# leopard-ai/betty

Hardware: AMD Instinct MI355X
Metric: hypergradient-steps/sec (CG K=20, 10M inner params) (higher is better)
Workload: dtype f32

## Files before the change

betty_amd/_native.py:

```python
from __future__ import annotations

import ctypes
import os
from ctypes import POINTER, c_char_p, c_double, c_float, c_int, c_int32, c_int64, c_size_t, c_void_p

_HERE = os.path.dirname(os.path.abspath(__file__))
LIB_PATH = os.environ.get("BHG_LIB") or os.path.join(_HERE, "csrc", "libbhg.so")
AB_LIB_PATH = os.environ.get("BHG_AB_LIB") or os.path.join(_HERE, "csrc", "libbhg_ab.so")

BHG_CHUNK_ELEMS = 4096
BHG_FLAT_ALIGN = 64
BHG_CG_AUTO, BHG_CG_STREAM, BHG_CG_RESIDENT = 0, 1, 2
BHG_CG_GLOBAL_CHAIN, BHG_CG_GLOBAL_UPDATE, BHG_CG_GLOBAL_DOTS = 0, 1, 2
BHG_CG_FX_BEGIN, BHG_CG_FX_CHAIN, BHG_CG_FX_GRAM, BHG_CG_FX_END = 0, 1, 2, 3


class NativeLibraryError(RuntimeError):
    """libbhg.so is missing or a call into it failed."""


class Chunk(ctypes.Structure):

    _fields_ = [
        ("flat_off", c_int64),
# ... 98 lines not shown
        c_int,
        [c_void_p, c_void_p, c_void_p, c_void_p, c_void_p, c_void_p, c_void_p, c_int, c_int, c_int, c_float, c_float, c_int, c_int, c_void_p],
    ),
    "bhg_logreg_neumann_solve": (
        c_int,
        [c_void_p, c_void_p, c_void_p, c_void_p, c_void_p, c_void_p, c_void_p, c_int, c_int, c_int, c_float, c_float, c_int, c_int, c_void_p],
    ),
    "bhg_mlp_partial_floats": (c_size_t, [POINTER(Mlp)]),
    "bhg_mlp_hvp": (c_int, [POINTER(Mlp), _PP, _PP, c_void_p]),
    "bhg_mlp_hvp_mode": (c_int, [POINTER(Mlp), _PP, _PP, c_int, c_void_p]),
    "bhg_mlp_supports_native_prepare": (c_int, [POINTER(Mlp)]),
    "bhg_mlp_forward": (c_int, [POINTER(Mlp), _PP, c_void_p, c_void_p, c_void_p]),
    "bhg_mlp_backward": (c_int, [POINTER(Mlp), c_void_p, c_void_p]),
    "bhg_mlp_mixed_coeff": (c_int, [POINTER(Mlp), _PP, c_void_p, c_void_p, c_void_p]),
    "bhg_mlp_supports_fused_solve": (c_int, [POINTER(Mlp)]),
    "bhg_mlp_fused_ws_bytes": (c_size_t, [POINTER(Mlp)]),
    "bhg_mlp_cg_solve": (
        c_int,
        [POINTER(Mlp), c_void_p, c_void_p, c_void_p, POINTER(c_int64), _CH, c_int, c_int, c_float, c_float, c_void_p,
         c_void_p, c_size_t, c_void_p],
    ),
    "bhg_mlp_cg_state_mask": (ctypes.c_uint64, [POINTER(Mlp), c_int]),
    "bhg_mlp_cg_solve_rhs": (
        c_int,
        [POINTER(Mlp), c_void_p, c_void_p, c_void_p, POINTER(c_int64), _CH, c_int, c_int, c_float, c_float, c_void_p,
         c_void_p, c_size_t, _PP, c_void_p],
    ),
    "bhg_mlp_cg_global_phase": (
        c_int,
        [POINTER(Mlp), c_void_p, c_void_p, c_void_p, POINTER(c_int64), _CH, c_int, c_int, c_int, c_int, c_int, c_void_p, c_float,
         c_float, c_void_p, c_void_p, c_size_t, c_void_p],
    ),
    "bhg_mlp_fx_supported": (c_int, [POINTER(Mlp), c_int]),
    "bhg_mlp_fx_ws_bytes": (c_size_t, [POINTER(Mlp), c_int]),
    "bhg_mlp_fx_const_floats": (c_size_t, [POINTER(Mlp)]),
    "bhg_mlp_fx_slab_floats": (c_size_t, [POINTER(Mlp)]),
    "bhg_mlp_fx_scal_doubles": (c_size_t, [POINTER(Mlp)]),
    "bhg_mlp_cg_fx_phase": (
        c_int,
        [POINTER(Mlp), _PP, c_int, c_int, c_int, c_int, c_int, c_void_p, c_void_p, c_void_p, c_float, c_float, c_void_p, c_size_t,
         c_void_p, c_size_t, c_void_p],
    ),
    "bhg_mlp_neumann_fx_phase": (
        c_int,
        [POINTER(Mlp), _PP, c_int, c_int, c_int, c_int, c_int, c_void_p, c_void_p, c_void_p, c_float, c_float, c_void_p, c_size_t,
         c_void_p, c_size_t, c_void_p],
    ),
    "bhg_mlp_cg_mixed_coeff": (c_int, [POINTER(Mlp), c_void_p, c_void_p, c_float, c_void_p, c_size_t, c_void_p]),
    "bhg_mlp_timeout_flag_dev": (c_void_p, [POINTER(Mlp), c_void_p]),
    "bhg_mlp_stage_batch": (c_int, [POINTER(Mlp), c_void_p, c_void_p, c_void_p, c_void_p]),
    "bhg_mlp_supports_packed_prepare": (c_int, [POINTER(Mlp)]),
    "bhg_mlp_forward_packed": (c_int, [POINTER(Mlp), _PP, c_void_p, c_void_p, c_void_p, c_size_t, c_void_p]),
    "bhg_mlp_backward_packed": (c_int, [POINTER(Mlp), c_void_p, c_void_p, c_size_t, c_void_p]),
    "bhg_mwn_max_hidden": (c_int, []),
    "bhg_mlp_fd_ws_bytes": (c_size_t, [POINTER(c_int), c_int, c_int]),
    "bhg_mlp_fd_forward": (
        c_int,
        [c_void_p, c_void_p, c_int, POINTER(c_int), c_int, _PP, _PP, c_void_p, c_int, c_void_p, c_void_p, c_void_p, c_size_t, c_void_p],
    ),
    "bhg_mwn_fd_vjp": (
        c_int,
        [c_void_p, c_void_p, c_int, c_void_p, c_void_p, c_void_p, c_void_p, c_int, c_void_p, c_int, c_void_p, c_void_p, c_void_p, c_void_p,
         c_void_p],
    ),
    "bhg_quad_fd": (c_int, [_PP, _PP, _PP, c_int, _CH, c_int, c_void_p, c_float, c_int, c_int, c_int, c_void_p]),
    "bhg_mwn_forward": (c_int, [c_void_p, c_int, c_void_p, c_void_p, c_void_p, c_void_p, c_int, c_void_p, c_void_p, c_void_p]),
    "bhg_mwn_backward": (
        c_int,
        [c_void_p, c_void_p, c_int, c_void_p, c_void_p, c_void_p, c_void_p, c_int, c_float, c_void_p, c_void_p, c_void_p, c_void_p, c_void_p],
    ),
    "bhg_mlp_neumann_solve": (
        c_int,
        [POINTER(Mlp), c_void_p, c_void_p, c_void_p, POINTER(c_int64), c_int, c_float, c_float, c_void_p, c_size_t, POINTER(c_int), c_void_p],
    ),
    "bhg_mlp_wsk_launches": (c_int64, []),
    "bhg_mlp_hoist_launches": (c_int64, []),
    "bhg_mlp_proj_iterations": (c_int64, []),
    "bhg_mlp_lin_launches": (c_int64, []),
    "bhg_mlp_neumann_mixed_coeff": (c_int, [POINTER(Mlp), _PP, c_void_p, c_void_p, c_float, c_int, c_int, c_void_p, c_size_t, c_void_p]),
    "bhg_mlp_plan_describe": (c_int, [POINTER(Mlp), c_int, c_int, ctypes.c_char_p, c_size_t]),
    "bhg_copy2d": (c_int, [c_void_p, c_int64, c_void_p, c_int64, c_int64, c_int64, c_void_p]),
    "bhg_bn_ws_bytes": (c_size_t, [c_int]),
    "bhg_bn_backward_vjp": (
        c_int,
        [c_void_p, c_void_p, c_void_p, c_void_p, c_void_p, c_void_p, c_void_p, c_void_p, c_int, c_int, c_int, c_void_p, c_void_p, c_void_p,
         c_void_p, c_size_t, c_void_p],
    ),
}

_libs = {}
_current = [None]


_PY_ENV = {"BHG_LIB", "BHG_AB_LIB", "BHG_HVP_GRAPH", "BHG_ALL_RANKS_ON_GPU0"}
_warned_env = [False]


def _warn_legacy_env() -> None:
    if _warned_env[0]:
        return
    _warned_env[0] = True
    stale = sorted(k for k in os.environ if k.startswith("BHG_") and k not in _PY_ENV)
    if stale:
        import warnings

        warnings.warn("betty_amd: environment variable(s) " + ", ".join(stale) + " are IGNORED — libbhg reads no environment variable. "
# ... 101 lines not shown
```

betty_amd/csrc/bhg_common.hpp:

```cpp
#pragma once
#include <hip/hip_runtime.h>
#include <stdint.h>
#include <stddef.h>
#include <stdio.h>
#include <string.h>

#include "bhg.h"

namespace bhg {

constexpr int kThreads = 256;
constexpr int kWaves = kThreads / 64;
constexpr int kChunk = BHG_CHUNK_ELEMS;
constexpr int kVecPerThread = kChunk / (kThreads * 4);
constexpr int kMaxBlocks = 1024;
constexpr int kInlineT = 32;
constexpr int kWriterT = 448;

constexpr size_t kWsScal = 0;
constexpr size_t kWsPartP = 128;
constexpr size_t kWsPartR = kWsPartP + 8 * kMaxBlocks;
constexpr size_t kWsBarrier = kWsPartR + 16 * kMaxBlocks;
constexpr size_t kWsTables = kWsBarrier + 256;
inline size_t ws_bytes(int T) {
  size_t b = kWsTables + 4 * sizeof(void*) * (size_t)(T > 0 ? T : 0);
  return (b + 255) & ~(size_t)255;
}

enum { S_RR_OLD = 0, S_PHP = 1, S_ALPHA = 2, S_RR_NEW = 3, S_BETA = 4, S_PP = 5 , S_ALPHA_RING = 10 ,
       S_NPART0 = 8  };

#define BHG_DBG_KEYS(X)                                                                                                      \
  X(mlp_wsk) X(mlp_wsk_maxk) X(mlp_wsk_depth) X(mlp_wsk_lds) X(wsl_depth) X(no_nt_slabs) X(gemm_no_xpose) X(mlp_no_fast)      \
  X(mlp_tn) X(split_target) X(split_cap) X(mlp_no_head) X(gram_ksplit) X(gram_kchunk) X(proj_graw_split) X(mlp_proj)         \
  X(mlp_hoist) X(hoist_wgs) X(proj_step_alone) X(mlp_no_side) X(mlp_no_fuse) X(mlp_no_outer_all) X(neumann_side)             \
  X(hoist_staged_mink) X(proj_alpha_alone) X(proj_small_alone) X(outer_order_by_work) X(outer_no_pre) X(outer_stagger)       \
  X(mlp_no_fused_solve) X(cg_eager_p) X(cg_x_every_iter) X(neumann_p_every_iter) X(head_no_prefetch) X(cg_spin_limit)        \
  X(packed_chain) X(packed_depth) X(packed_gram) X(proj_max_ratio) X(proj_ws_cap_mb) X(alpha_in_hoist) X(graw_v2) X(wskp_ragged) X(pstep_v2) X(pstep_unroll) X(rnew_in_graw) X(graw_cols) X(lin_first) X(lin_prio) X(lin_nub) X(lin_order) X(lin_update_next) X(lin_withhold_beta) X(neumann_vnew) X(cg_rhs_direct) X(packed_prepare) X(lin_deep) X(graw_kloop) X(lin_update_in_head) X(xcd_pairs) X(headu_head_first) X(fx_ksplit)
enum DbgKey : int {
#define BHG_DBG_ENUM(n) DBG_##n,
  BHG_DBG_KEYS(BHG_DBG_ENUM)
#undef BHG_DBG_ENUM
  DBG_COUNT
};
constexpr int kDbgUnset = INT32_MIN;
#ifdef BHG_AB
extern int g_dbg[DBG_COUNT];
inline bool dbg_is_set(DbgKey k) { return g_dbg[k] != kDbgUnset; }
inline int dbg(DbgKey k, int dflt) { return g_dbg[k] == kDbgUnset ? dflt : g_dbg[k]; }
#else
constexpr bool dbg_is_set(DbgKey) { return false; }
constexpr int dbg(DbgKey, int dflt) { return dflt; }
#endif

constexpr int kStampKernels = 4, kStampBlocks = 4096, kStampSlots = 8;
#ifdef BHG_STAMPS
#ifdef __HIPCC__
#define BHG_STAMP(kid, slot)                                                                                            \
  do {                                                                                                                  \
    if (threadIdx.x == 0 && blockIdx.x < ::bhg::kStampBlocks) {                                                         \
      unsigned long long* sp_ = ::bhg::d_stamps;                                                                        \
      if (sp_) sp_[((kid) * ::bhg::kStampBlocks + blockIdx.x) * ::bhg::kStampSlots + (slot)] = wall_clock64();          \
    }                                                                                                                   \
  } while (0)
#endif
#else
#define BHG_STAMP(kid, slot) do { } while (0)
#endif

void set_error(const char* fmt, ...);
#define BHG_HIP_CHECK(expr)                                                        \
  do {                                                                             \
    hipError_t _e = (expr);                                                        \
    if (_e != hipSuccess) {                                                        \
      ::bhg::set_error("%s failed: %s (%s:%d)", #expr, hipGetErrorString(_e), __FILE__, \
                       __LINE__);                                                  \
      return BHG_ERR_HIP;                                                          \
    }                                                                              \
  } while (0)
#define BHG_REQUIRE(cond, msg)                                                     \
  do {                                                                             \
    if (!(cond)) {                                                                 \
      ::bhg::set_error("%s: %s", __func__, msg);                                   \
      return BHG_ERR_ARG;                                                          \
    }                                                                              \
  } while (0)

struct PtrTab {
  const void* const* dev;
  const void* inl[kInlineT];
};

int make_table(PtrTab* out, const void* const* host_ptrs, int T, void* ws, int slot,
               hipStream_t stream);

bool span_begin(int kind, hipEvent_t* a, hipEvent_t* b);

#ifdef __HIPCC__
__device__ __forceinline__ float* tab_ptr(const PtrTab& t, int i) {
  const void* p = t.dev ? t.dev[i] : t.inl[i];
  return (float*)p;
}

__device__ __forceinline__ float4 ld4(const float* __restrict__ base, int e, int len) {
  if (e + 4 <= len) return *reinterpret_cast<const float4*>(base + e);
  float4 r = make_float4(0.f, 0.f, 0.f, 0.f);
  if (e < len) r.x = base[e];
  if (e + 1 < len) r.y = base[e + 1];
  if (e + 2 < len) r.z = base[e + 2];
  return r;
}
__device__ __forceinline__ void st4(float* __restrict__ base, int e, int len, float4 v) {
  if (e + 4 <= len) {
    *reinterpret_cast<float4*>(base + e) = v;
    return;
  }
  if (e < len) base[e] = v.x;
  if (e + 1 < len) base[e + 1] = v.y;
  if (e + 2 < len) base[e + 2] = v.z;
}

template <int BYTES>
__device__ __forceinline__ void kernarg_warm() {
  typedef const __attribute__((address_space(4))) unsigned* KP;
  KP kp = (KP)__builtin_amdgcn_kernarg_segment_ptr();
  unsigned acc = 0;
#pragma unroll
  for (int o = 0; o < BYTES; o += 64) acc |= kp[o / 4];
  asm volatile("" ::"s"(acc));
}
template <int U>
__device__ __forceinline__ double sum_strided(const double* __restrict__ p, const int n, const int t, const int stride) {
  double acc = 0.0;
  for (int i0 = t; i0 < n; i0 += U * stride) {
    double v[U];
#pragma unroll
    for (int u = 0; u < U; ++u) {
      const int i = i0 + u * stride;
      v[u] = p[i < n ? i : n - 1];
    }
#pragma unroll
    for (int u = 0; u < U; ++u)
      if (i0 + u * stride < n) acc += v[u];
  }
  return acc;
}

template <int U>
struct StridedRegs { double v[U]; };
template <int U>
// ... 87 lines not shown
```

betty_amd/csrc/bhg_mlp.hip:

```cpp
#include <stdlib.h>
#include <vector>


#include "bhg_common.hpp"

#ifdef BHG_STAMPS
namespace bhg { __device__ unsigned long long* d_stamps = nullptr; }
#endif

namespace bhg {
namespace {
#include "mlp/gemm.inc"

#include "mlp/outer.inc"

#include "mlp/scalars.inc"

#include "mlp/head.inc"

#include "mlp/wsk.inc"

#include "mlp/wskp.inc"

inline int wsk_mode(int chain_mode, int unfused_hint) {
// ... 2015 lines not shown

int bhg_mlp_backward_packed(const bhg_mlp* m, const int64_t* labels, void* fws, size_t fws_bytes, void* stream) {
  if (int rc = check_head_problem(m)) return rc;
  BHG_REQUIRE(narrow_head(m), "the packed once-per-step passes need a narrow classifier head (<= 256 classes, feature width % 4 == 0)");
  BHG_REQUIRE(labels && fws, "NULL argument");
  BHG_REQUIRE(bhg_mlp_supports_packed_prepare(m), "this network does not take the packed form (bhg_mlp_supports_packed_prepare)");
  BHG_REQUIRE(fws_bytes >= bhg_mlp_fused_ws_bytes(m), "fused workspace too small");
  hipStream_t st = static_cast<hipStream_t>(stream);
  const int L = m->L, Bp = m->Bp, B = m->B;
  const int C = m->dims[L];
  FusedWs w;
  carve_fused_ws(m, fws, &w);
  hipLaunchKernelGGL(k_delta_top, dim3((Bp * C + 255) / 256), dim3(256), 0, st, m->prob, m->sd, labels,
                     const_cast<float*>(m->delta[L - 1]), Bp, C, B);
  {
    const int l = L - 1, K = m->dims[l + 1], N = m->dims[l];
    const int blocks = (Bp * (N / 4) + 255) / 256;
    hipLaunchKernelGGL(k_head_backward, dim3(blocks), dim3(256), 0, st, (const float*)nullptr, m->delta[l], m->W[l],
                       (const float*)nullptr, m->mask[l - 1], const_cast<float*>(m->delta[l - 1]), N, K, B, Bp, w.dpk[l - 1]);
  }
  for (int l = L - 2; l >= 1; --l) {
    WskpBuilder wb;
    WskpProb q{};
    q.Ap = w.dpk[l]; q.Bq = w.Wb[l]; q.RA = Bp; q.RB = m->dims[l]; q.K = m->dims[l + 1]; q.B = B; q.nsplit = 1;
    q.mask = m->mask[l - 1]; q.out = const_cast<float*>(m->delta[l - 1]);
    q.outp = l >= 2 ? w.dpk[l - 1] : nullptr;
    wb.add(q);
    wb.launch(st);
  }
  BHG_HIP_CHECK(hipGetLastError());
  return BHG_OK;
}

__global__ __launch_bounds__(256) void k_stage_batch(const float* __restrict__ x, const int64_t* __restrict__ y, float* __restrict__ h0,
                                                     int64_t* __restrict__ labels, int64_t n4, int B) {
  for (int64_t i = (int64_t)blockIdx.x * 256 + threadIdx.x; i < n4; i += (int64_t)gridDim.x * 256)
    reinterpret_cast<float4*>(h0)[i] = reinterpret_cast<const float4*>(x)[i];
  if (blockIdx.x == 0)
    for (int b = threadIdx.x; b < B; b += 256) labels[b] = y[b];
}
int bhg_mlp_stage_batch(const bhg_mlp* m, const float* x, const int64_t* y, int64_t* labels, void* stream) {
  if (int rc = check_mlp(m)) return rc;
  BHG_REQUIRE(x && y && labels && m->h[0], "NULL argument");
  BHG_REQUIRE((m->dims[0] & 3) == 0 && ((uintptr_t)x & 15) == 0, "the input batch must be 16-byte aligned with a width that is a multiple of 4");
  const int64_t n4 = (int64_t)m->B * m->dims[0] / 4;
  int blocks = (int)((n4 + 255) / 256);
  if (blocks > 2048) blocks = 2048;
  if (blocks < 1) blocks = 1;
  hipLaunchKernelGGL(k_stage_batch, dim3(blocks), dim3(256), 0, static_cast<hipStream_t>(stream), x, y, const_cast<float*>(m->h[0]), labels, n4, m->B);
  BHG_HIP_CHECK(hipGetLastError());
  return BHG_OK;
}

int bhg_mlp_mixed_coeff(const bhg_mlp* m, const void* const* dir, const int64_t* labels, float* coeff, void* stream) {
  if (int rc = check_head_problem(m)) return rc;
  BHG_REQUIRE(dir && labels && coeff, "NULL argument");
  hipStream_t st = static_cast<hipStream_t>(stream);
  const int L = m->L, Bp = m->Bp, B = m->B;
  for (int l = 0; l < L; ++l) {
    const int K = m->dims[l], N = m->dims[l + 1];
    const float* V = static_cast<const float*>(dir[2 * l]);
    const float* c = static_cast<const float*>(dir[2 * l + 1]);
    if (l == L - 1 && narrow_head(m)) {
      launch_head_forward(st, Bp, l > 0 ? (const float*)m->Rh[l - 1] : nullptr, m->h[l], m->W[l], V, c, m->prob, nullptr,
                          nullptr, K, N, B, HEAD_COEFF, labels, coeff, nullptr, nullptr, nullptr);
      break;
    }
    GemmArgs a{};
    a.pr[0] = {m->h[l], V, K, K};
    a.pairs = 1;
    if (l > 0) { a.pr[1] = {m->Rh[l - 1], m->W[l], K, K}; a.pairs = 2; }
    a.M = Bp; a.N = N; a.K = K;
    const int tn = skinny_tile_n();
    a.splits = pick_splits((N + tn - 1) / tn, K, a.pairs);
    a.out = m->partial; a.ldo = N; a.out_rows = Bp;
    launch_gemm<LAYOUT_KC, LAYOUT_KC>(a, tn, st);
    if (l == L - 1) {
      launch_reduce_mask(st, m->partial, a.splits, Bp * N, c, nullptr, m->Rd[l], Bp, N, B);
      hipLaunchKernelGGL(k_coeff_rows, dim3(Bp), dim3(kThreads), 0, st, m->prob, (const float*)m->Rd[l], labels, coeff, N, B);
      break;
    }
    launch_reduce_mask(st, m->partial, a.splits, Bp * N, c, m->mask[l], m->Rh[l], Bp, N, B);
  }
  BHG_HIP_CHECK(hipGetLastError());
  return BHG_OK;
}

int bhg_mlp_plan_describe(const bhg_mlp* m, int algo, int keep_solution, char* buf, size_t buf_bytes) {
  if (int rc = check_mlp(m)) return rc;
  BHG_REQUIRE(buf && buf_bytes >= 64, "output buffer too small");
  BHG_REQUIRE(algo == 0 || algo == 1, "algo: 0 = cg, 1 = neumann");
  const int L = m->L;
  const bool fused = bhg_mlp_supports_fused_solve(m) != 0;
  HoistPlan hp;
  hoist_plan(m, &hp);
  const char* form = "unfused";
  int hoist = 0, proj_level = 0, lin = 0, lin_head = 0, upd_first = 0;
  const char* closing = "k_outer_all";
  if (fused) {
    int64_t numel[2 * BHG_MLP_MAX_LAYERS], starts[2 * BHG_MLP_MAX_LAYERS];
    for (int l = 0; l < L; ++l) { numel[2 * l] = (int64_t)m->dims[l] * m->dims[l + 1]; numel[2 * l + 1] = m->dims[l + 1]; }
    const int64_t nch = bhg_layout_num_chunks(numel, 2 * L);
    std::vector<bhg_chunk> chunks((size_t)(nch > 0 ? nch : 1));
    if (int rc = bhg_layout_build(numel, 2 * L, starts, chunks.data())) return rc;
    float* const fake = reinterpret_cast<float*>((uintptr_t)1 << 30);
    if (algo == 0) {
      static CgCtx c;
      cg_ctx_init(&c, m, keep_solution ? fake : nullptr, fake, fake, starts, nullptr, (int)nch, 2, 1.f, 0.f, fake, fake, false);
      hoist = c.hoist ? 1 : 0; proj_level = c.proj_level; lin = c.lin ? 1 : 0; lin_head = c.lin_head ? 1 : 0;
      upd_first = (c.lin && L > 4) ? 1 : 0;
      form = !c.lazy ? "classic-eager" : (!c.hoist ? "classic" : (c.proj_level == 0 ? "hoisted" : (c.proj_level == 1 ? "projected-keep-state" :
             (c.lin ? (c.lin_head ? "six-launch (k_wskpl .. k_headu .. k_graw)" : "six-launch-class (k_wskpl first, recurrences beside the chain)") :
              "fully-projected (k_pstep launch)"))));
      if (c.proj_level >= 1) closing = graw_batch_ok(m->Bp) ? (m->Bp == 128 ? "k_graw" : "k_grawk") : "k_hoist+k_proj_update";
    } else {
      const bool want_proj = !keep_solution && proj_mode() != 0 && hoist_mode() != 0;
      const bool proj = want_proj && hp.ok && hp.proj_ok && use_head(m);
      hoist = (hp.ok && (hoist_mode() == 2 || want_proj)) ? 1 : 0;
      proj_level = proj ? 1 : 0;
      form = proj ? "projected-neumann (update inside k_graw)" : (hoist ? "hoisted" : "classic");
      if (proj) closing = graw_batch_ok(m->Bp) ? (m->Bp == 128 ? "k_graw" : "k_grawk") : "k_hoist+k_proj_update";
    }
  }
  size_t gram = 0;
  if (hp.ok && hp.proj_ok)
    for (int l = 0; l + 1 < L; ++l) gram += (size_t)m->Bp * m->Bp * (l >= 1 ? (2 + 2 * kGramSplitMax + 6) : 2);
  const int n = snprintf(buf, buf_bytes,
                         "algo=%s keep_solution=%d fused=%d form=\"%s\" hoist=%d proj_level=%d lin=%d lin_head=%d upd_first=%d closing=%s "
                         "plan_ok=%d proj_ok=%d lin_ok=%d hoist_products=%d hoist_wgs=%d gram_floats=%zu fused_ws_bytes=%zu narrow_head=%d packed_prepare=%d "
                         "global_form=%s fx_slab_bytes=%zu fx_ws_bytes_world8=%zu",
                         algo == 0 ? "cg" : "neumann", keep_solution ? 1 : 0, fused ? 1 : 0, form, hoist, proj_level, lin, lin_head, upd_first, closing,
                         hp.ok ? 1 : 0, hp.proj_ok ? 1 : 0, hp.lin_ok ? 1 : 0, hp.n, hp.ok ? hp.blk0[hp.n] : 0, gram,
                         fused ? bhg_mlp_fused_ws_bytes(m) : (size_t)0, narrow_head(m) ? 1 : 0, bhg_mlp_supports_packed_prepare(m),
                         (algo == 0 && !keep_solution && bhg_mlp_fx_supported(m, 1)) ? "factor-exchange" : (fused ? "one-pass" : "sharded"),
                         sizeof(float) * bhg_mlp_fx_slab_floats(m), bhg_mlp_fx_ws_bytes(m, 8));
  BHG_REQUIRE(n > 0 && (size_t)n < buf_bytes, "output buffer too small");
  return BHG_OK;
}

#ifdef BHG_STAMPS
static unsigned long long* g_stamps_dev = nullptr;
int bhg_debug_stamps_enable(int on) {
  const size_t bytes = sizeof(unsigned long long) * bhg::kStampKernels * bhg::kStampBlocks * bhg::kStampSlots;
  if (on && !g_stamps_dev) {
    BHG_HIP_CHECK(hipMalloc(&g_stamps_dev, bytes));
  }
  if (g_stamps_dev) BHG_HIP_CHECK(hipMemset(g_stamps_dev, 0, bytes));
  unsigned long long* p = on ? g_stamps_dev : nullptr;
  BHG_HIP_CHECK(hipMemcpyToSymbol(HIP_SYMBOL(bhg::d_stamps), &p, sizeof(p)));
  return BHG_OK;
}
int bhg_debug_stamps_read(unsigned long long* host, size_t count) {
  BHG_REQUIRE(g_stamps_dev && host, "stamps are not enabled");
  const size_t total = (size_t)bhg::kStampKernels * bhg::kStampBlocks * bhg::kStampSlots;
  BHG_HIP_CHECK(hipDeviceSynchronize());
  BHG_HIP_CHECK(hipMemcpy(host, g_stamps_dev, sizeof(unsigned long long) * (count < total ? count : total), hipMemcpyDeviceToHost));
  return BHG_OK;
}
#endif

}

#ifndef BHG_LAYOUT_PAD
#define BHG_LAYOUT_PAD 8
#endif
namespace bhg {
namespace {
#define BHG_STR2(x) #x
#define BHG_STR(x) BHG_STR2(x)
__global__ __attribute__((aligned(16384))) void k_layout_anchor() {
#if BHG_LAYOUT_PAD > 0
  asm volatile(".rept " BHG_STR(BHG_LAYOUT_PAD) " * 64 - 8\n s_nop 0\n .endr");
#endif
}
}
}
```

betty_amd/hypergradient/_mlp_hip.py:

```python
from __future__ import annotations

import ctypes
import weakref

import torch

from .. import _native

TILE_M = 128

_BUFFERS = weakref.WeakKeyDictionary()



class _Buffers:

    def __init__(self, dims, BP, device, lib):
        L = len(dims) - 1
        self.BP = BP
        self.dims, self.L = dims, L
        z = lambda *shape: torch.zeros(*shape, dtype=torch.float32, device=device)
        self.h = [z(BP, dims[l]) for l in range(L)]
        self.mask = [z(BP, dims[l + 1]) for l in range(L - 1)]
        self.delta = [z(BP, dims[l + 1]) for l in range(L)]
# ... 56 lines not shown
    __slots__ = ("kind", "alpha", "K", "layout", "v_last", "materialised", "projected")

    def __init__(self, kind, alpha, K, layout, v_last=None, materialised=True, projected=0):
        self.kind, self.alpha, self.K, self.layout, self.v_last, self.materialised = kind, alpha, K, layout, v_last, materialised
        self.projected = projected

    def __bool__(self):
        return True


class HipMLPState:
    def __init__(self, spec, x, y):
        if not x.is_cuda:
            raise _native.NativeLibraryError("WeightedCEMLP(impl='hip') needs CUDA/HIP tensors; there is no CPU fallback")
        self.lib = lib = _native.load()
        self.spec = spec
        Ws = [lin.weight.detach() for lin in spec.layers]
        bs = [lin.bias.detach() for lin in spec.layers]
        L, B = len(Ws), x.shape[0]
        BP = (B + TILE_M - 1) // TILE_M * TILE_M
        if L > _native.BHG_MLP_MAX_LAYERS:
            raise ValueError("too many layers")
        for t in Ws + bs:
            if t.dtype != torch.float32 or not t.is_contiguous() or t.data_ptr() % 16 != 0:
                raise ValueError("weights and biases must be contiguous, 16-byte aligned fp32 tensors")
        dims = tuple([Ws[0].shape[1]] + [W.shape[0] for W in Ws])
        key = (dims, BP, str(x.device))
        owner = _BUFFERS.setdefault(spec.layers[0], {})
        buf = owner.get(key)
        if buf is None:
            buf = owner[key] = _Buffers(dims, BP, x.device, lib)
        self.buf, self.B, self.L, self.Ws = buf, B, L, Ws
        d = buf.desc
        d.B = B
        for l in range(L):
            d.W[l] = Ws[l].data_ptr()
        self.desc = d
        if getattr(buf, "last_B", B) > B:
            buf.h[0][B:].zero_()
        buf.last_B = B
        xs, ys = x.detach().reshape(B, -1), y.detach().reshape(-1)
        same_dev = (xs.device == buf.h[0].device and ys.device == xs.device and xs.is_cuda
                    and torch.cuda.current_device() == (xs.device.index if xs.device.index is not None else torch.cuda.current_device()))
        if (same_dev and xs.dtype == torch.float32 and xs.is_contiguous() and xs.data_ptr() % 16 == 0 and dims[0] % 4 == 0
                and ys.dtype == torch.int64 and ys.is_contiguous()):
            _native.check(lib.bhg_mlp_stage_batch(ctypes.byref(d), xs.data_ptr(), ys.data_ptr(), buf.labels.data_ptr(), _stream()),
                          "bhg_mlp_stage_batch")
        else:
            buf.h[0][:B].copy_(xs.to(torch.float32))
            buf.labels[:B].copy_(ys)

        d.prepacked = 0
        self.packed_prepare = bool(buf.native_prepare and lib.bhg_mlp_supports_packed_prepare(ctypes.byref(d)))
        if self.packed_prepare:
            fws = self._fused_ws(x.device)
            bias_tab, self._bias_keep = _native.ptr_array([b.data_ptr() for b in bs])
            _native.check(lib.bhg_mlp_forward_packed(ctypes.byref(d), bias_tab, buf.labels.data_ptr(), buf.ce.data_ptr(), fws.data_ptr(),
                                                     fws.numel(), _stream()), "bhg_mlp_forward_packed")
            ce = buf.ce[:B]
        elif buf.native_prepare:
            bias_tab, self._bias_keep = _native.ptr_array([b.data_ptr() for b in bs])
            _native.check(lib.bhg_mlp_forward(ctypes.byref(d), bias_tab, buf.labels.data_ptr(), buf.ce.data_ptr(), _stream()),
                          "bhg_mlp_forward")
            ce = buf.ce[:B]
        else:
            raise _native.NativeLibraryError("bhg_mlp_supports_native_prepare refused this network (layer count / batch padding): there is no ATen path")
        native = _native_weight_net(lib, spec.weight_net, spec.prev.trainable_parameters(), x.device)
        self.native_upper, self.sample_weight = native is not None, None
        if self.native_upper:
            self._wn, self._upper_slots = native
            ts = self._wn
            _native.check(lib.bhg_mwn_forward(buf.ce.data_ptr(), B, ts[0].data_ptr(), ts[1].data_ptr(), ts[2].data_ptr(), ts[3].data_ptr(),
                                              ts[0].shape[0], None, buf.sd.data_ptr(), _stream()), "bhg_mwn_forward")
        else:
            self.sample_weight = spec.weight_fn(ce.detach().clone())
            buf.sd[:B].copy_(self.sample_weight.detach().reshape(-1).to(torch.float32) / B)
        if self.packed_prepare:
            _native.check(lib.bhg_mlp_backward_packed(ctypes.byref(d), buf.labels.data_ptr(), buf.fws.data_ptr(), buf.fws.numel(), _stream()),
                          "bhg_mlp_backward_packed")
            d.prepacked = 1
        else:
            _native.check(lib.bhg_mlp_backward(ctypes.byref(d), buf.labels.data_ptr(), _stream()), "bhg_mlp_backward")
        if buf.out is None:
            buf.out = []
            for lin in spec.layers:
                buf.out += [torch.empty_like(lin.weight), torch.empty_like(lin.bias)]
            buf.out_tab, buf.out_keep = _native.ptr_array([t.data_ptr() for t in buf.out])
        self.out = buf.out
        self._out_tab = buf.out_tab

    def upper_vjp(self, coeff, upper, scale: float = 1.0, retain_graph: bool = False, with_flat: bool = False):
        if not self.native_upper:
            sw = self.sample_weight
            out = list(torch.autograd.grad(sw, upper, grad_outputs=coeff.reshape(sw.shape), retain_graph=retain_graph, allow_unused=retain_graph))
            return (out, None) if with_flat else out
        ts, B = self._wn, self.B
        H = ts[0].shape[0]
        flat, views, g = _flat_upper(upper, self._upper_slots, ts[0].device)
        coeff = coeff if (coeff.dtype == torch.float32 and coeff.is_contiguous()) else coeff.to(torch.float32).contiguous()
        _native.check(
            self.lib.bhg_mwn_backward(self.buf.ce.data_ptr(), coeff.data_ptr(), B, ts[0].data_ptr(), ts[1].data_ptr(), ts[2].data_ptr(),
                                      ts[3].data_ptr(), H, float(scale), g[0].data_ptr(), g[1].data_ptr(), g[2].data_ptr(),
                                      g[3].data_ptr(), _stream()), "bhg_mwn_backward")
        return (views, flat) if with_flat else views

    @staticmethod
    def _dir_table(direction_views):
        dirs = []
        for t in direction_views:
            if not (t.is_cuda and t.dtype == torch.float32 and t.is_contiguous() and t.data_ptr() % 16 == 0):
                t = t.detach().to(torch.float32).contiguous().clone()
            dirs.append(t)
        tab, keep = _native.ptr_array([t.data_ptr() for t in dirs])
        return tab, (dirs, keep)

    def hvp(self, direction_views):
        self._solve = None
        key = tuple(map(id, direction_views))
        cached = getattr(self, "_dir_cache", None)
        if cached is None or cached[0] != key:
            tab, keep = self._dir_table(direction_views)
            cached = (key, tab, keep, list(direction_views))
            self._dir_cache = cached if all(a is b for a, b in zip(keep[0], direction_views)) else None
        mode = 3 if getattr(getattr(self.spec.curr, "config", None), "type", None) == "neumann" else 0
        _native.check(self.lib.bhg_mlp_hvp_mode(ctypes.byref(self.desc), cached[1], self._out_tab, mode, _stream()), "bhg_mlp_hvp_mode")
        return self.out

    def fused_supported(self, layout) -> bool:
        if not self.lib.bhg_mlp_supports_fused_solve(ctypes.byref(self.desc)):
            return False
        want = []
        for W in self.Ws:
            want += [W.numel(), W.shape[0]]
        return tuple(want) == tuple(layout.numels) and str(layout.device) == str(self.Ws[0].device)

# ... 363 lines not shown
```

include/bhg.h:

```cpp
#ifndef BHG_H_
#define BHG_H_

#include <stddef.h>
#include <stdint.h>

#ifdef __cplusplus
extern "C" {
#endif

#define BHG_VERSION 1
#define BHG_CHUNK_ELEMS 4096
#define BHG_FLAT_ALIGN 64

#define BHG_OK 0
#define BHG_ERR_ARG (-1)
#define BHG_ERR_HIP (-2)
#define BHG_ERR_WS (-3)
#define BHG_ERR_CAPACITY (-4)

typedef struct bhg_chunk {
  int64_t flat_off;
  int64_t src_off;
  int32_t tensor;
  int32_t len;
// ... 110 lines not shown

int bhg_mlp_supports_native_prepare(const bhg_mlp* m);
int bhg_mlp_forward(const bhg_mlp* m, const void* const* bias, const int64_t* labels, float* ce, void* stream);
int bhg_mlp_backward(const bhg_mlp* m, const int64_t* labels, void* stream);
int bhg_mlp_mixed_coeff(const bhg_mlp* m, const void* const* dir, const int64_t* labels, float* coeff, void* stream);

int bhg_mlp_supports_fused_solve(const bhg_mlp* m);
size_t bhg_mlp_fused_ws_bytes(const bhg_mlp* m);
int bhg_mlp_cg_solve(const bhg_mlp* m, float* x, float* r, float* p, const int64_t* starts,
                     const bhg_chunk* chunks_dev, int n_chunks, int K, float cg_alpha, float hvp_shift, void* ws,
                     void* fws, size_t fws_bytes, void* stream);
int bhg_mlp_neumann_solve(const bhg_mlp* m, float* v0, float* v1, float* p, const int64_t* starts, int K,
                          float alpha, float hvp_shift, void* fws, size_t fws_bytes, int* projected_out, void* stream);
#define BHG_CG_GLOBAL_CHAIN 0
#define BHG_CG_GLOBAL_UPDATE 1
#define BHG_CG_GLOBAL_DOTS 2
int bhg_mlp_cg_global_phase(const bhg_mlp* m, float* x, float* r, float* p, const int64_t* starts, const bhg_chunk* chunks_dev,
                            int n_chunks, int k, int K, int phase, int world, double* php, float cg_alpha, float hvp_shift,
                            void* ws, void* fws, size_t fws_bytes, void* stream);
#define BHG_CG_FX_BEGIN 0
#define BHG_CG_FX_CHAIN 1
#define BHG_CG_FX_GRAM 2
#define BHG_CG_FX_END 3
int bhg_mlp_fx_supported(const bhg_mlp* m, int world);
size_t bhg_mlp_fx_ws_bytes(const bhg_mlp* m, int world);
size_t bhg_mlp_fx_const_floats(const bhg_mlp* m);
size_t bhg_mlp_fx_slab_floats(const bhg_mlp* m);
size_t bhg_mlp_fx_scal_doubles(const bhg_mlp* m);
int bhg_mlp_cg_fx_phase(const bhg_mlp* m, const void* const* rhs, int k, int K, int phase, int world, int rank, float* const_all,
                        float* slab_all, double* scal_all, float cg_alpha, float hvp_shift, void* fws, size_t fws_bytes, void* xws,
                        size_t xws_bytes, void* stream);
int bhg_mlp_neumann_fx_phase(const bhg_mlp* m, const void* const* rhs, int k, int K, int phase, int world, int rank, float* const_all,
                             float* slab_all, double* scal_all, float alpha, float hvp_shift, void* fws, size_t fws_bytes, void* xws,
                             size_t xws_bytes, void* stream);
unsigned long long bhg_mlp_cg_state_mask(const bhg_mlp* m, int has_x);
int bhg_mlp_cg_solve_rhs(const bhg_mlp* m, float* x, float* r, float* p, const int64_t* starts, const bhg_chunk* chunks_dev,
                         int n_chunks, int K, float cg_alpha, float hvp_shift, void* ws, void* fws, size_t fws_bytes,
                         const void* const* rhs, void* stream);
int bhg_mlp_cg_mixed_coeff(const bhg_mlp* m, const int64_t* labels, float* coeff, float cg_alpha, void* fws,
                           size_t fws_bytes, void* stream);
int64_t bhg_mlp_wsk_launches(void);
int64_t bhg_mlp_hoist_launches(void);
int64_t bhg_mlp_proj_iterations(void);
int64_t bhg_mlp_lin_launches(void);
int bhg_mlp_neumann_mixed_coeff(const bhg_mlp* m, const void* const* v_last, const int64_t* labels, float* coeff,
                                float alpha, int K, int projected, void* fws, size_t fws_bytes, void* stream);

int bhg_mlp_stage_batch(const bhg_mlp* m, const float* x, const int64_t* y, int64_t* labels, void* stream);
int bhg_mlp_supports_packed_prepare(const bhg_mlp* m);
int bhg_mlp_forward_packed(const bhg_mlp* m, const void* const* bias, const int64_t* labels, float* ce, void* fws, size_t fws_bytes,
                           void* stream);
int bhg_mlp_backward_packed(const bhg_mlp* m, const int64_t* labels, void* fws, size_t fws_bytes, void* stream);

void* bhg_mlp_timeout_flag_dev(const bhg_mlp* m, void* fws);

int bhg_mwn_max_hidden(void);
int bhg_mwn_forward(const float* ce, int B, const float* w1, const float* b1, const float* w2, const float* b2, int H, float* s,
                    float* sd, void* stream);
int bhg_mwn_backward(const float* ce, const float* coeff, int B, const float* w1, const float* b1, const float* w2, const float* b2,
                     int H, float scale, float* gw1, float* gb1, float* gw2, float* gb2, void* stream);

int bhg_mlp_plan_describe(const bhg_mlp* m, int algo, int keep_solution, char* buf, size_t buf_bytes);

int bhg_copy2d(float* dst, int64_t ldd, const float* src, int64_t lds, int64_t rows, int64_t cols, void* stream);

size_t bhg_bn_ws_bytes(int C);
int bhg_bn_backward_vjp(const float* x, const float* gy, const float* a, const float* gamma, const float* mean, const float* invstd,
                        const float* b, const float* c, int N, int C, int HW, float* dx, float* dgy, float* dgamma, void* ws,
                        size_t ws_bytes, void* stream);

size_t bhg_mlp_fd_ws_bytes(const int* dims, int L, int B);
int bhg_mlp_fd_forward(const float* x, const int64_t* labels, int B, const int* dims, int L, void* const* params, const void* const* dir,
                       const float* eps_dev, int restore, float* ce_plus, float* ce_minus, void* ws, size_t ws_bytes, void* stream);
int bhg_mwn_fd_vjp(const float* ce_plus, const float* ce_minus, int B, const float* w1, const float* b1, const float* w2, const float* b2,
                   int H, const float* two_eps_dev, int accumulate, float* gw1, float* gb1, float* gw2, float* gb2, void* stream);

int bhg_quad_fd(void* const* w, const void* const* dir, void* const* out, int T, const bhg_chunk* chunks_dev, int n_chunks,
                const float* eps_dev, float scale, int mode, int restore, int accumulate, void* stream);

#ifdef __cplusplus
}
#endif
#endif
```

Baseline: 768.1.

## Fuse classifier head, softmax-CE, weight-net forward and first backward layer into one kernel

Adds a per-sample kernel that computes the last-layer logits, softmax, cross-entropy, the meta weight-net forward (sample weight), the top delta and the masked delta for the previous layer. It also writes that delta in packed form. This replaces separate forward-head, mwn_forward and backward-head launches in the once-per-step prepare phase, cutting kernel launches and round trips through global memory. The cost is a restricted shape envelope (C<=12, K<=1024, H<=2048) and serial per-sample softmax and weight-net math in one thread.

Measured after the change: 770.9, median of 5. About the same (+0.4%).

```diff
diff --git a/betty_amd/_native.py b/betty_amd/_native.py
--- a/betty_amd/_native.py
+++ b/betty_amd/_native.py
@@ -174,6 +174,11 @@
     "bhg_mlp_supports_packed_prepare": (c_int, [POINTER(Mlp)]),
     "bhg_mlp_forward_packed": (c_int, [POINTER(Mlp), _PP, c_void_p, c_void_p, c_void_p, c_size_t, c_void_p]),
     "bhg_mlp_backward_packed": (c_int, [POINTER(Mlp), c_void_p, c_void_p, c_size_t, c_void_p]),
+    "bhg_mlp_supports_fused_tail": (c_int, [POINTER(Mlp), c_int]),
+    "bhg_mlp_prepare_packed": (
+        c_int,
+        [POINTER(Mlp), _PP, c_void_p, c_void_p, c_void_p, c_void_p, c_void_p, c_void_p, c_int, c_void_p, c_size_t, c_void_p],
+    ),
     "bhg_mwn_max_hidden": (c_int, []),
     "bhg_mlp_fd_ws_bytes": (c_size_t, [POINTER(c_int), c_int, c_int]),
     "bhg_mlp_fd_forward": (
diff --git a/betty_amd/csrc/bhg_common.hpp b/betty_amd/csrc/bhg_common.hpp
--- a/betty_amd/csrc/bhg_common.hpp
+++ b/betty_amd/csrc/bhg_common.hpp
@@ -36,7 +36,7 @@
   X(mlp_hoist) X(hoist_wgs) X(proj_step_alone) X(mlp_no_side) X(mlp_no_fuse) X(mlp_no_outer_all) X(neumann_side)             \
   X(hoist_staged_mink) X(proj_alpha_alone) X(proj_small_alone) X(outer_order_by_work) X(outer_no_pre) X(outer_stagger)       \
   X(mlp_no_fused_solve) X(cg_eager_p) X(cg_x_every_iter) X(neumann_p_every_iter) X(head_no_prefetch) X(cg_spin_limit)        \
-  X(packed_chain) X(packed_depth) X(packed_gram) X(proj_max_ratio) X(proj_ws_cap_mb) X(alpha_in_hoist) X(graw_v2) X(wskp_ragged) X(pstep_v2) X(pstep_unroll) X(rnew_in_graw) X(graw_cols) X(lin_first) X(lin_prio) X(lin_nub) X(lin_order) X(lin_update_next) X(lin_withhold_beta) X(neumann_vnew) X(cg_rhs_direct) X(packed_prepare) X(lin_deep) X(graw_kloop) X(lin_update_in_head) X(xcd_pairs) X(headu_head_first) X(fx_ksplit)
+  X(packed_chain) X(packed_depth) X(packed_gram) X(proj_max_ratio) X(proj_ws_cap_mb) X(alpha_in_hoist) X(graw_v2) X(wskp_ragged) X(pstep_v2) X(pstep_unroll) X(rnew_in_graw) X(graw_cols) X(lin_first) X(lin_prio) X(lin_nub) X(lin_order) X(lin_update_next) X(lin_withhold_beta) X(neumann_vnew) X(cg_rhs_direct) X(packed_prepare) X(lin_deep) X(graw_kloop) X(lin_update_in_head) X(xcd_pairs) X(headu_head_first) X(fx_ksplit) X(fused_tail)
 enum DbgKey : int {
 #define BHG_DBG_ENUM(n) DBG_##n,
   BHG_DBG_KEYS(BHG_DBG_ENUM)
@@ -96,6 +96,17 @@
 
 bool span_begin(int kind, hipEvent_t* a, hipEvent_t* b);
 
+struct PrepareTailArgs {
+  const float* h; const float* W; const float* bias;
+  const int64_t* labels;
+  const float* w1; const float* b1; const float* w2; const float* b2; int H;
+  float* prob; float* ce; float* sd; float* delta_top;
+  const float* mask_prev; float* delta_prev; float* delta_prev_p;
+  int K, C, B, rows;
+};
+bool prepare_tail_takes(int K, int C, int H);
+int launch_prepare_tail(const PrepareTailArgs& a, hipStream_t st);
+
 #ifdef __HIPCC__
 __device__ __forceinline__ float* tab_ptr(const PtrTab& t, int i) {
   const void* p = t.dev ? t.dev[i] : t.inl[i];
diff --git a/betty_amd/csrc/bhg_mlp.hip b/betty_amd/csrc/bhg_mlp.hip
--- a/betty_amd/csrc/bhg_mlp.hip
+++ b/betty_amd/csrc/bhg_mlp.hip
@@ -2091,6 +2091,70 @@
   return BHG_OK;
 }
 
+int bhg_mlp_supports_fused_tail(const bhg_mlp* m, int H) {
+  if (!bhg_mlp_supports_packed_prepare(m) || dbg(DBG_fused_tail, 1) == 0) return 0;
+  return narrow_head(m) && prepare_tail_takes(m->dims[m->L - 1], m->dims[m->L], H) ? 1 : 0;
+}
+int bhg_mlp_prepare_packed(const bhg_mlp* m, const void* const* bias, const int64_t* labels, float* ce,
+                           const float* w1, const float* b1, const float* w2, const float* b2, int H, void* fws, size_t fws_bytes,
+                           void* stream) {
+  if (int rc = check_head_problem(m)) return rc;
+  BHG_REQUIRE(narrow_head(m), "the packed once-per-step passes need a narrow classifier head (<= 256 classes, feature width % 4 == 0)");
+  BHG_REQUIRE(bias && labels && ce && fws, "NULL argument");
+  BHG_REQUIRE(bhg_mlp_supports_packed_prepare(m), "this network does not take the packed form (bhg_mlp_supports_packed_prepare)");
+  BHG_REQUIRE(fws_bytes >= bhg_mlp_fused_ws_bytes(m), "fused workspace too small");
+  BHG_REQUIRE(w1 && b1 && w2 && b2 && m->sd && bhg_mlp_supports_fused_tail(m, H), "this head / weight net does not take the fused tail (bhg_mlp_supports_fused_tail)");
+  hipStream_t st = static_cast<hipStream_t>(stream);
+  const int L = m->L, Bp = m->Bp, B = m->B;
+  FusedWs w;
+  carve_fused_ws(m, fws, &w);
+  if (int rc = pack_operands(m, w, st, true)) return rc;
+  {
+    const int K = m->dims[0], N = m->dims[1];
+    GemmArgs a{};
+    a.pr[0] = {m->h[0], m->W[0], K, K};
+    a.pairs = 1;
+    a.M = Bp; a.N = N; a.K = K;
+    const int tn = skinny_tile_n();
+    a.splits = pick_splits((N + tn - 1) / tn, K, 1);
+    a.out = m->partial; a.ldo = N; a.out_rows = Bp;
+    launch_gemm<LAYOUT_KC, LAYOUT_KC>(a, tn, st);
+    launch_reduce_mask(st, m->partial, a.splits, Bp * N, static_cast<const float*>(bias[0]), nullptr, const_cast<float*>(m->h[1]), Bp, N, B,
+                       const_cast<float*>(m->mask[0]), w.hpk[1]);
+  }
+  for (int l = 1; l + 1 < L; ++l) {
+    WskpfArgs f{};
+    WskpProb& q = f.a;
+    q.Ap = w.hpk[l]; q.Bq = w.Wf[l]; q.RA = Bp; q.RB = m->dims[l + 1]; q.K = m->dims[l]; q.B = B; q.nsplit = 1;
+    q.bias = static_cast<const float*>(bias[l]);
+    q.out = const_cast<float*>(m->h[l + 1]);
+    q.outp = l + 2 < L ? w.hpk[l + 1] : nullptr;
+    f.relu_mask = const_cast<float*>(m->mask[l]);
+    wskp_tiling(&q, false);
+    const int blk = q.nfull * (q.RB / 32) + q.nstrip;
+    hipLaunchKernelGGL(k_wskpf<2>, dim3(blk), dim3(64 * kWskpWaves), 0, st, f);
+  }
+  PrepareTailArgs t{};
+  t.h = m->h[L - 1]; t.W = m->W[L - 1]; t.bias = static_cast<const float*>(bias[L - 1]);
+  t.labels = labels;
+  t.w1 = w1; t.b1 = b1; t.w2 = w2; t.b2 = b2; t.H = H;
+  t.prob = const_cast<float*>(m->prob); t.ce = ce; t.sd = const_cast<float*>(m->sd); t.delta_top = const_cast<float*>(m->delta[L - 1]);
+  t.mask_prev = m->mask[L - 2]; t.delta_prev = const_cast<float*>(m->delta[L - 2]); t.delta_prev_p = w.dpk[L - 2];
+  t.K = m->dims[L - 1]; t.C = m->dims[L]; t.B = B; t.rows = Bp;
+  if (int rc = launch_prepare_tail(t, st)) return rc;
+  for (int l = L - 2; l >= 1; --l) {
+    WskpBuilder wb;
+    WskpProb q{};
+    q.Ap = w.dpk[l]; q.Bq = w.Wb[l]; q.RA = Bp; q.RB = m->dims[l]; q.K = m->dims[l + 1]; q.B = B; q.nsplit = 1;
+    q.mask = m->mask[l - 1]; q.out = const_cast<float*>(m->delta[l - 1]);
+    q.outp = l >= 2 ? w.dpk[l - 1] : nullptr;
+    wb.add(q);
+    wb.launch(st);
+  }
+  BHG_HIP_CHECK(hipGetLastError());
+  return BHG_OK;
+}
+
 int bhg_mlp_mixed_coeff(const bhg_mlp* m, const void* const* dir, const int64_t* labels, float* coeff, void* stream) {
   if (int rc = check_head_problem(m)) return rc;
   BHG_REQUIRE(dir && labels && coeff, "NULL argument");
@@ -2167,10 +2231,11 @@
   const int n = snprintf(buf, buf_bytes,
                          "algo=%s keep_solution=%d fused=%d form=\"%s\" hoist=%d proj_level=%d lin=%d lin_head=%d upd_first=%d closing=%s "
                          "plan_ok=%d proj_ok=%d lin_ok=%d hoist_products=%d hoist_wgs=%d gram_floats=%zu fused_ws_bytes=%zu narrow_head=%d packed_prepare=%d "
-                         "global_form=%s fx_slab_bytes=%zu fx_ws_bytes_world8=%zu",
+                         "fused_tail=%d global_form=%s fx_slab_bytes=%zu fx_ws_bytes_world8=%zu",
                          algo == 0 ? "cg" : "neumann", keep_solution ? 1 : 0, fused ? 1 : 0, form, hoist, proj_level, lin, lin_head, upd_first, closing,
                          hp.ok ? 1 : 0, hp.proj_ok ? 1 : 0, hp.lin_ok ? 1 : 0, hp.n, hp.ok ? hp.blk0[hp.n] : 0, gram,
                          fused ? bhg_mlp_fused_ws_bytes(m) : (size_t)0, narrow_head(m) ? 1 : 0, bhg_mlp_supports_packed_prepare(m),
+                         bhg_mlp_supports_fused_tail(m, 1),
                          (algo == 0 && !keep_solution && bhg_mlp_fx_supported(m, 1)) ? "factor-exchange" : (fused ? "one-pass" : "sharded"),
                          sizeof(float) * bhg_mlp_fx_slab_floats(m), bhg_mlp_fx_ws_bytes(m, 8));
   BHG_REQUIRE(n > 0 && (size_t)n < buf_bytes, "output buffer too small");
diff --git a/betty_amd/csrc/bhg_prepare.hip b/betty_amd/csrc/bhg_prepare.hip
--- /dev/null
+++ b/betty_amd/csrc/bhg_prepare.hip
@@ -0,0 +1,131 @@
+#include "bhg_common.hpp"
+
+namespace bhg {
+namespace {
+
+constexpr int kTailMaxC = 12;
+constexpr int kTailMaxK = 1024;
+constexpr int kTailMaxH = 2048;
+
+__device__ __forceinline__ float4 ldv(const float* p) { return *reinterpret_cast<const float4*>(p); }
+
+__global__ __launch_bounds__(256) void k_prepare_tail(const PrepareTailArgs a) {
+  extern __shared__ float sp[];
+  __shared__ float rz[kTailMaxC], pr[kTailMaxC], dl[kTailMaxC];
+  __shared__ float s_sd;
+  const int b = blockIdx.x, t = threadIdx.x;
+  const int lane = t & 63, wave = t >> 6;
+  const int K = a.K, C = a.C, B = a.B, H = a.H, rows = a.rows;
+  const int k4 = 4 * t;
+  if (b >= B) {
+    if (t < C) { a.prob[(int64_t)b * C + t] = 0.f; a.delta_top[(int64_t)b * C + t] = 0.f; }
+    if (t == 0) a.ce[b] = 0.f;
+    if (k4 < K) {
+      const float4 z = make_float4(0.f, 0.f, 0.f, 0.f);
+      *reinterpret_cast<float4*>(a.delta_prev + (int64_t)b * K + k4) = z;
+      *reinterpret_cast<float4*>(a.delta_prev_p + ((int64_t)(k4 >> 4) * rows + b) * 16 + (k4 & 15)) = z;
+    }
+    return;
+  }
+  const float* hb = a.h + (int64_t)b * K;
+  constexpr int JMAX = 3;
+  float acc[JMAX], cbv[JMAX];
+  const float* wrow[JMAX];
+#pragma unroll
+  for (int j = 0; j < JMAX; ++j) {
+    const int cc = min(wave + 4 * j, C - 1);
+    acc[j] = 0.f;
+    wrow[j] = a.W + (int64_t)cc * K;
+    cbv[j] = a.bias[cc];
+  }
+  const int kd = k4 < K ? k4 : 0;
+  const float4 pf_mk = ldv(a.mask_prev + (int64_t)b * K + kd);
+  float4 pf_W[kTailMaxC];
+#pragma unroll
+  for (int c = 0; c < kTailMaxC; ++c) pf_W[c] = ldv(a.W + (int64_t)min(c, C - 1) * K + kd);
+  const int y = (int)a.labels[b];
+  const float bias2 = a.b2[0];
+  for (int j = t; j < H; j += 256) { sp[j] = a.w1[j]; sp[H + j] = a.b1[j]; sp[2 * H + j] = a.w2[j]; }
+  for (int k = 4 * lane; k < K; k += 256) {
+    const float4 hv = ldv(hb + k);
+    float4 vv[JMAX];
+#pragma unroll
+    for (int j = 0; j < JMAX; ++j) vv[j] = ldv(wrow[j] + k);
+#pragma unroll
+    for (int j = 0; j < JMAX; ++j) {
+      float s = acc[j];
+      s = fmaf(hv.x, vv[j].x, s); s = fmaf(hv.y, vv[j].y, s); s = fmaf(hv.z, vv[j].z, s); s = fmaf(hv.w, vv[j].w, s);
+      acc[j] = s;
+    }
+  }
+#pragma unroll
+  for (int j = 0; j < JMAX; ++j) {
+    const int c = wave + 4 * j;
+    const float s = wave_sum_f32(acc[j]);
+    if (lane == 0 && c < C) rz[c] = s + cbv[j];
+  }
+  __syncthreads();
+  if (t == 0) {
+    float mx = rz[0];
+    for (int c = 1; c < C; ++c) mx = fmaxf(mx, rz[c]);
+    float sum = 0.f;
+    for (int c = 0; c < C; ++c) sum += expf(rz[c] - mx);
+    const float lse = mx + logf(sum);
+    for (int c = 0; c < C; ++c) {
+      const float p = expf(rz[c] - lse);
+      a.prob[(int64_t)b * C + c] = p;
+      pr[c] = p;
+    }
+    const float ce = lse - rz[y];
+    a.ce[b] = ce;
+    float z = bias2;
+    for (int j = 0; j < H; ++j) {
+      const float u = fmaf(sp[j], ce, sp[H + j]);
+      z = fmaf(sp[2 * H + j], u > 0.f ? u : 0.f, z);
+    }
+    const float v = 1.f / (1.f + expf(-z));
+    const float sdv = v / (float)B;
+    a.sd[b] = sdv;
+    s_sd = sdv;
+  }
+  __syncthreads();
+  if (t < C) {
+    const float d = s_sd * (pr[t] - (y == t ? 1.f : 0.f));
+    a.delta_top[(int64_t)b * C + t] = d;
+    dl[t] = d;
+  }
+  __syncthreads();
+  if (k4 < K) {
+    float4 s = make_float4(0.f, 0.f, 0.f, 0.f);
+#pragma unroll
+    for (int c = 0; c < kTailMaxC; ++c) {
+      if (c < C) {
+        const float r = dl[c];
+        const float4 w = pf_W[c];
+        s.x += r * w.x; s.y += r * w.y; s.z += r * w.z; s.w += r * w.w;
+      }
+    }
+    s.x *= pf_mk.x; s.y *= pf_mk.y; s.z *= pf_mk.z; s.w *= pf_mk.w;
+    *reinterpret_cast<float4*>(a.delta_prev + (int64_t)b * K + k4) = s;
+    *reinterpret_cast<float4*>(a.delta_prev_p + ((int64_t)(k4 >> 4) * rows + b) * 16 + (k4 & 15)) = s;
+  }
+}
+
+}
+
+bool prepare_tail_takes(int K, int C, int H) {
+  return C >= 1 && C <= kTailMaxC && K >= 16 && K <= kTailMaxK && (K & 15) == 0 && H >= 1 && H <= kTailMaxH;
+}
+
+int launch_prepare_tail(const PrepareTailArgs& a, hipStream_t st) {
+  BHG_REQUIRE(prepare_tail_takes(a.K, a.C, a.H), "this head / weight net is outside what the fused tail takes (prepare_tail_takes)");
+  BHG_REQUIRE(a.h && a.W && a.bias && a.labels && a.w1 && a.b1 && a.w2 && a.b2 && a.prob && a.ce && a.sd && a.delta_top && a.mask_prev &&
+                  a.delta_prev && a.delta_prev_p,
+              "NULL argument");
+  BHG_REQUIRE(a.rows >= a.B && a.B >= 1, "rows must cover the batch");
+  hipLaunchKernelGGL(k_prepare_tail, dim3(a.rows), dim3(256), sizeof(float) * 3 * (size_t)a.H, st, a);
+  BHG_HIP_CHECK(hipGetLastError());
+  return BHG_OK;
+}
+
+}
diff --git a/betty_amd/hypergradient/_mlp_hip.py b/betty_amd/hypergradient/_mlp_hip.py
--- a/betty_amd/hypergradient/_mlp_hip.py
+++ b/betty_amd/hypergradient/_mlp_hip.py
@@ -132,11 +132,23 @@
 
         d.prepacked = 0
         self.packed_prepare = bool(buf.native_prepare and lib.bhg_mlp_supports_packed_prepare(ctypes.byref(d)))
+        native = _native_weight_net(lib, spec.weight_net, spec.prev.trainable_parameters(), x.device)
+        self.native_upper, self.sample_weight = native is not None, None
+        if self.native_upper:
+            self._wn, self._upper_slots = native
+        H = self._wn[0].shape[0] if self.native_upper else 0
+        self.fused_tail = bool(self.packed_prepare and self.native_upper and lib.bhg_mlp_supports_fused_tail(ctypes.byref(d), H))
         if self.packed_prepare:
             fws = self._fused_ws(x.device)
             bias_tab, self._bias_keep = _native.ptr_array([b.data_ptr() for b in bs])
-            _native.check(lib.bhg_mlp_forward_packed(ctypes.byref(d), bias_tab, buf.labels.data_ptr(), buf.ce.data_ptr(), fws.data_ptr(),
-                                                     fws.numel(), _stream()), "bhg_mlp_forward_packed")
+            if self.fused_tail:
+                ts = self._wn
+                _native.check(lib.bhg_mlp_prepare_packed(ctypes.byref(d), bias_tab, buf.labels.data_ptr(), buf.ce.data_ptr(), ts[0].data_ptr(),
+                                                         ts[1].data_ptr(), ts[2].data_ptr(), ts[3].data_ptr(), H, fws.data_ptr(), fws.numel(),
+                                                         _stream()), "bhg_mlp_prepare_packed")
+            else:
+                _native.check(lib.bhg_mlp_forward_packed(ctypes.byref(d), bias_tab, buf.labels.data_ptr(), buf.ce.data_ptr(), fws.data_ptr(),
+                                                         fws.numel(), _stream()), "bhg_mlp_forward_packed")
             ce = buf.ce[:B]
         elif buf.native_prepare:
             bias_tab, self._bias_keep = _native.ptr_array([b.data_ptr() for b in bs])
@@ -145,22 +157,22 @@
             ce = buf.ce[:B]
         else:
             raise _native.NativeLibraryError("bhg_mlp_supports_native_prepare refused this network (layer count / batch padding): there is no ATen path")
-        native = _native_weight_net(lib, spec.weight_net, spec.prev.trainable_parameters(), x.device)
-        self.native_upper, self.sample_weight = native is not None, None
-        if self.native_upper:
-            self._wn, self._upper_slots = native
-            ts = self._wn
-            _native.check(lib.bhg_mwn_forward(buf.ce.data_ptr(), B, ts[0].data_ptr(), ts[1].data_ptr(), ts[2].data_ptr(), ts[3].data_ptr(),
-                                              ts[0].shape[0], None, buf.sd.data_ptr(), _stream()), "bhg_mwn_forward")
-        else:
-            self.sample_weight = spec.weight_fn(ce.detach().clone())
-            buf.sd[:B].copy_(self.sample_weight.detach().reshape(-1).to(torch.float32) / B)
-        if self.packed_prepare:
-            _native.check(lib.bhg_mlp_backward_packed(ctypes.byref(d), buf.labels.data_ptr(), buf.fws.data_ptr(), buf.fws.numel(), _stream()),
-                          "bhg_mlp_backward_packed")
+        if self.fused_tail:
             d.prepacked = 1
         else:
-            _native.check(lib.bhg_mlp_backward(ctypes.byref(d), buf.labels.data_ptr(), _stream()), "bhg_mlp_backward")
+            if self.native_upper:
+                ts = self._wn
+                _native.check(lib.bhg_mwn_forward(buf.ce.data_ptr(), B, ts[0].data_ptr(), ts[1].data_ptr(), ts[2].data_ptr(), ts[3].data_ptr(),
+                                                  ts[0].shape[0], None, buf.sd.data_ptr(), _stream()), "bhg_mwn_forward")
+            else:
+                self.sample_weight = spec.weight_fn(ce.detach().clone())
+                buf.sd[:B].copy_(self.sample_weight.detach().reshape(-1).to(torch.float32) / B)
+            if self.packed_prepare:
+                _native.check(lib.bhg_mlp_backward_packed(ctypes.byref(d), buf.labels.data_ptr(), buf.fws.data_ptr(), buf.fws.numel(), _stream()),
+                              "bhg_mlp_backward_packed")
+                d.prepacked = 1
+            else:
+                _native.check(lib.bhg_mlp_backward(ctypes.byref(d), buf.labels.data_ptr(), _stream()), "bhg_mlp_backward")
         if buf.out is None:
             buf.out = []
             for lin in spec.layers:
diff --git a/include/bhg.h b/include/bhg.h
--- a/include/bhg.h
+++ b/include/bhg.h
@@ -186,6 +186,10 @@
                            void* stream);
 int bhg_mlp_backward_packed(const bhg_mlp* m, const int64_t* labels, void* fws, size_t fws_bytes, void* stream);
 
+int bhg_mlp_supports_fused_tail(const bhg_mlp* m, int H);
+int bhg_mlp_prepare_packed(const bhg_mlp* m, const void* const* bias, const int64_t* labels, float* ce, const float* w1, const float* b1,
+                           const float* w2, const float* b2, int H, void* fws, size_t fws_bytes, void* stream);
+
 void* bhg_mlp_timeout_flag_dev(const bhg_mlp* m, void* fws);
 
 int bhg_mwn_max_hidden(void);
```
